# ShuoYangRobotics/Cerberus

Hardware: NVIDIA H100
Metric: sliding-window solves/sec (10-frame x 150-feature windows) (higher is better)
Workload: dtype f64

## Files before the change

cerberus_b200/csrc/solve_kernel.cuh:

```cuda
#pragma once
#include "eval_kernels.cuh"

namespace cerb {

#if defined(CERB_PHASE_TIMING) && !defined(CERB_CUSIM)
__device__ unsigned long long g_phase_cycles[48];
#define PH_DECL() long long ph_t = clock64()
#define PH_MARK_T(id, t) do { if ((threadIdx.x & 31) == 0) { const long long ph_n = clock64(); if (threadIdx.x == (t)) atomicAdd(&g_phase_cycles[id], (unsigned long long)(ph_n - ph_t)); ph_t = ph_n; } __syncwarp(); } while (0)
#define PH_MARK(id) PH_MARK_T(id, 0)
#define PH_ARG , long long &ph_t
#define PH_FWD , ph_t
#else
#define PH_DECL()
#define PH_MARK_T(id, t)
#define PH_MARK(id)
#define PH_ARG
#define PH_FWD
#endif

enum { CERB_WINDOW = 10, NX = 79, NYB = 13, NFR = 11, NY = 143, NR = 222, NRP = 224, HXX_SZ = 79 * 79, HXY_SZ = 79 * 143, X_TD = 78, SOLVE_THREADS = 256, FT = 64, TILE_LD = 33, NOBS_PLANES = 9 };
enum { HBLK = NYB * NYB, AD_SZ = NFR * HBLK, BO_SZ = (NFR - 1) * HBLK };
#ifndef CERB_SOLVE_MIN_BLOCKS
#define CERB_SOLVE_MIN_BLOCKS 1
#endif
enum { PIMG_HXY = HXX_SZ + 1, PIMG_REST = HXY_SZ + AD_SZ + BO_SZ, PIMG_SZ = PIMG_HXY + PIMG_REST, SMEM_HXX_PAD = 3 };
static_assert((PIMG_HXY * 8) % 16 == 0 && (PIMG_REST * 8) % 16 == 0 && ((HXX_SZ + SMEM_HXX_PAD) * 8) % 16 == 0, "bulk-copy alignment of the prior image");

struct SolveParams {
    int n_windows, maxF, maxObs, max_iters, optimize_leg_bias;
    double G[3], sqrt_info, huber;
    double radius0, max_radius, min_radius, min_rel_dec, ftol, gtol, ptol;
    const int *n_features, *feat_start, *feat_nobs, *feat_off, *flags;
    const double *obs; const int *obs_stereo;
    const double *pre;
    const double *sinfo;
    const double *prior_J, *prior_r, *prior_x0, *prior_Hp; const int *prior_meta;
    double *state, *lam;
    int *rep_i; double *rep_d;
    double *ws;
    long ws_stride;
    double *dbg; int dbg_window;
    double test_initial_mu;
    int no_bulk_copy;
    int test_fail_factorizations;
};

CERB_HD long ws_vecs(int F) { return (long)NX * F; }
CERB_HD long ws_prior(int F) { return (long)NX * F + 9L * F; }
CERB_HD long ws_chunks(int F) { return ws_prior(F) + PIMG_SZ; }
CERB_HD long ws_imuplan(int F) { return (ws_chunks(F) + (F + 4) / 2 + 8 + 1) & ~1L; }
CERB_HD long ws_size(int F) { return ws_imuplan(F) + 15 * 2 * 32 * 4 / 2 + 8; }
struct CtaWs {
    double *W, *hh, *gl, *sl, *Dl, *ghl, *gnl, *stl, *lamc, *sinv;
    int *chunks;
    int *imu_plan;
    double *pimg;
    int F;
};
CERB_D CtaWs ws_carve(const SolveParams &P) {
    double *ws = P.ws + (size_t)blockIdx.x * P.ws_stride;
    const int F = P.maxF;
    CtaWs v;
    v.W = ws;
    v.hh = ws + ws_vecs(F); v.gl = v.hh + F; v.sl = v.gl + F; v.Dl = v.sl + F; v.ghl = v.Dl + F; v.gnl = v.ghl + F; v.stl = v.gnl + F; v.lamc = v.stl + F; v.sinv = v.lamc + F;
    v.chunks = reinterpret_cast<int *>(ws + ws_chunks(F)); v.imu_plan = reinterpret_cast<int *>(ws + ws_imuplan(F));
    v.pimg = ws + ws_prior(F); v.F = F;
    return v;
}

struct Smem {
    double *Hxx, *Hxy, *Ad, *Bo;
    double *g, *sc, *D, *gh, *gn, *stp, *yv;
    double *xs, *xc;
    double *Rw, *Rex;
    double *Ju;
    double *lin;
    double *pdx, *pr;
    double *red;
    double *wj;
    double *sca;
    double *chain_col;
    double *idg;
    double *idx;
    int *ti;
    unsigned long long *mbar;
    double *tile;
};
enum { S_RADIUS = 0, S_MU, S_REUSE, S_XCOST, S_CCOST, S_ALPHA, S_GNORM2, S_GNNORM2, S_GDOTGN, S_MODEL, S_STEPNORM, S_XNORM, S_DLNORM,
       S_OK, S_DONE, S_TERM, S_ITER, S_NSUCC, S_INVALID, S_GMAX, S_INIT_COST, S_P, S_Q, S_VHV, S_LCOST, S_LNORM, S_LGMAX, S_COUNT };
static_assert(S_COUNT <= 32, "scalar slots overlap the chain's column line");
enum { TI_PRIOR_MAP = 0, TI_NCHUNKS = 96, TI_CHUNK_CACHE = 97, TI_CACHED_CHUNKS = 15, TI_CHAIN_DONE = 130, TI_IMU_MASK = 131, TI_INTS = 132 };
static_assert(TI_PRIOR_MAP + CERB_MAX_PRIOR_DIM <= TI_NCHUNKS && TI_CHUNK_CACHE + 2 * TI_CACHED_CHUNKS <= TI_CHAIN_DONE && TI_IMU_MASK < TI_INTS && TI_INTS % 2 == 0,
              "s.ti slots overlap");
enum { SMEM_DOUBLES = HXX_SZ + SMEM_HXX_PAD + HXY_SZ + AD_SZ + BO_SZ + 7 * NRP + 2 * ST_STRIDE + 99 + 18 + 3 + 31 * 39 + 960 + 192 + 8 * 256 + 128 * 8 + 32 + 32 + TI_INTS / 2 + 144 + 80 };

CERB_D void smem_carve(double *base, Smem &s) {
    double *p = base;
    s.Hxx = p; p += HXX_SZ; s.mbar = reinterpret_cast<unsigned long long *>(p + 1); p += SMEM_HXX_PAD; s.Hxy = p; p += HXY_SZ; s.Ad = p; p += AD_SZ; s.Bo = p; p += BO_SZ;
    s.g = p; p += NRP; s.sc = p; p += NRP; s.D = p; p += NRP; s.gh = p; p += NRP; s.gn = p; p += NRP; s.stp = p; p += NRP; s.yv = p; p += NRP;
    s.xs = p; p += ST_STRIDE; s.xc = p; p += ST_STRIDE;
    s.Rw = p; p += 99; s.Rex = p; p += 18; p += 3;
    s.Ju = p; p += 31 * 39; s.red = p; p += 8 * 256; s.wj = p; p += 128 * 8;
    s.lin = p; p += 960; s.pdx = p; p += 96; s.pr = p; p += 96; s.sca = p; p += 32; s.chain_col = p; p += 32;
    s.ti = reinterpret_cast<int *>(p); p += TI_INTS / 2;
    s.idg = p; p += 144;
    s.idx = p; p += 80;
    s.tile = s.Hxy;
}

template <int NV>
CERB_D void block_sum(const double *v, double *red, double *out, int tid) {
    for (int k = 0; k < NV; k++) red[k * 256 + tid] = v[k];
    __syncthreads();
    for (int s = 128; s > 0; s >>= 1) {
        if (tid < s) for (int k = 0; k < NV; k++) red[k * 256 + tid] += red[k * 256 + tid + s];
        __syncthreads();
    }
    for (int k = 0; k < NV; k++) out[k] = red[k * 256];
    __syncthreads();
}

CERB_D void copy_g2s(double *dst, const double *src, int n, int tid) {
    for (int k0 = tid; k0 < n; k0 += 8 * SOLVE_THREADS) {
        double b[8];
        _Pragma("unroll")
        for (int u = 0; u < 8; u++) { const int k = k0 + u * SOLVE_THREADS; b[u] = (k < n) ? src[k] : 0.0; }
        _Pragma("unroll")
        for (int u = 0; u < 8; u++) { const int k = k0 + u * SOLVE_THREADS; if (k < n) dst[k] = b[u]; }
    }
}
CERB_D void copy_g2s_async(double *dst, const double *src, int n, int tid) {
    for (int k = tid; k < n; k += SOLVE_THREADS) CERB_CP_ASYNC8(dst + k, src + k);
}
CERB_D void load_geometry(const double *x, Smem &s, int tid) {
    if (tid < 11) { const m33 R = qtoR(ldq(x + ST_POSE + 7 * tid + 3)); for (int k = 0; k < 9; k++) s.Rw[9 * tid + k] = R.m[k]; }
    else if (tid < 13) { const int e = tid - 11; const m33 R = qtoR(ldq(x + ST_EX + 7 * e + 3)); for (int k = 0; k < 9; k++) s.Rex[9 * e + k] = R.m[k]; }
    __syncthreads();
}

struct ObsCtx { int start, nobs, off; double lam, pix, piy, vix, viy, tdi; };

struct ObsVals { double px, py, vx, vy, td; int stereo; };
CERB_D void obs_fetch(const double *obs, const int *stereo, int mo, int o, int cam, ObsVals &v) {
    v.px = obs[(cam ? 4 : 0) * mo + o]; v.py = obs[(cam ? 5 : 1) * mo + o]; v.vx = obs[(cam ? 6 : 2) * mo + o]; v.vy = obs[(cam ? 7 : 3) * mo + o];
    v.td = obs[8 * mo + o]; v.stereo = stereo[o];
}

CERB_NOINLINE double vision_cost(const SolveParams &P, int w, const double *x, const double *lam, int tid) {
    CERB_DYN_SMEM(double, smem_base);
// ... 243 lines not shown
                        for (int ks = par; ks < nkt; ks += 2) {
                            const int rn = rb1 + 4 * (ks + 2 - par);
                            const bool more = ks + 2 < nkt;
                            const double n0 = more ? tq[0][rn] : 0.0, n1 = (more && !k3 && tv[1]) ? tq[1][rn] : 0.0, n2 = (more && tv[2]) ? tq[2][rn] : 0.0, n3 = (more && tv[3]) ? tq[3][rn] : 0.0;
                            CERB_DMMA(acc[0][0], acc[0][1], v0, v0, acc[0][0], acc[0][1]);
                            CERB_DMMA(acc[2][0], acc[2][1], v0, v2, acc[2][0], acc[2][1]);
                            CERB_DMMA(acc[3][0], acc[3][1], v0, v3, acc[3][0], acc[3][1]);
                            CERB_DMMA(acc[7][0], acc[7][1], v2, v2, acc[7][0], acc[7][1]);
                            CERB_DMMA(acc[8][0], acc[8][1], v2, v3, acc[8][0], acc[8][1]);
                            CERB_DMMA(acc[9][0], acc[9][1], v3, v3, acc[9][0], acc[9][1]);
                            if (!k3) {
                                CERB_DMMA(acc[1][0], acc[1][1], v0, v1, acc[1][0], acc[1][1]);
                                CERB_DMMA(acc[4][0], acc[4][1], v1, v1, acc[4][0], acc[4][1]);
                                CERB_DMMA(acc[5][0], acc[5][1], v1, v2, acc[5][0], acc[5][1]);
                                CERB_DMMA(acc[6][0], acc[6][1], v1, v3, acc[6][0], acc[6][1]);
                            }
                            v0 = n0; v1 = n1; v2 = n2; v3 = n3;
                        }
                    }
                    PH_MARK(28);
                    const int o = (lane >> 2) * 8 + 2 * (lane & 3);
                    pp[0 * 64 + o] += acc[0][0]; pp[0 * 64 + o + 1] += acc[0][1];
                    pp[1 * 64 + o] += acc[2][0]; pp[1 * 64 + o + 1] += acc[2][1];
                    pp[2 * 64 + o] += acc[3][0]; pp[2 * 64 + o + 1] += acc[3][1];
                    pp[3 * 64 + o] += acc[7][0]; pp[3 * 64 + o + 1] += acc[7][1];
                    pp[4 * 64 + o] += acc[8][0]; pp[4 * 64 + o + 1] += acc[8][1];
                    pp[5 * 64 + o] += acc[9][0]; pp[5 * 64 + o + 1] += acc[9][1];
                }
                {
                    const int o = wid * VJ_SZ + (lane >> 2) * 8 + 2 * (lane & 3);
                    jp[o] = acc[1][0]; jp[o + 1] = acc[1][1];
                    jp[64 + o] = acc[4][0]; jp[64 + o + 1] = acc[4][1];
                    jp[128 + o] = acc[5][0]; jp[128 + o + 1] = acc[5][1];
                    jp[192 + o] = acc[6][0]; jp[192 + o + 1] = acc[6][1];
                }
            }
            if (wrow && cam == 1) for (int k = 0; k < 6; k++) W[(size_t)(6 * j + k) * F + f] = wprev[k] + wjv[k] * (prescale ? s.sc[6 * j + k] * slf : 1.0);
            PH_MARK(29);
            __syncthreads();
            PH_MARK(22);
            if (jbase >= 0) {
                _Pragma("unroll")
                for (int fj = 0; fj < 2; fj++) {
                    const int jf = j0 + fj;
                    if (jf >= NFR || jf == a) continue;
                    const double *q = jp + (4 * fj) * VJ_SZ + tid;
                    smem_base[jbase + jca * a + jcj * jf] += ((q[0] + q[VJ_SZ]) + q[2 * VJ_SZ]) + q[3 * VJ_SZ];
                }
            }
            PH_MARK(23);
        }
        __syncthreads();
        {
            double *ex = T;
            ex[0 * 256 + tid] = h; ex[1 * 256 + tid] = gq; ex[2 * 256 + tid] = wT;
            for (int k = 0; k < 6; k++) { ex[(3 + k) * 256 + tid] = wI[k]; ex[(9 + k) * 256 + tid] = wE0[k]; ex[(15 + k) * 256 + tid] = wE1[k]; }
        }
        __syncthreads();
        for (int e = tid; e < VP_SZ; e += SOLVE_THREADS) {
            double v = 0.0;
            for (int wq = 0; wq < 8; wq++) v += ((wq < 5) ? s.Ju + 8 * VJ_SZ + VP_SZ * wq : s.tile + VT_SZ + VP_SZ * (wq - 5))[e];
            const int blk = e >> 6, ra = (e >> 3) & 7, rb = e & 7;
            const int ga = blk < 3 ? 0 : (blk < 5 ? 2 : 3), gb = blk == 0 ? 0 : (blk == 1 || blk == 3 ? 2 : 3);
            vis_scatter(s, ga, gb, ra, rb, a, a, v);
        }
        if (tid < 64 && ev) {
            const double *ex = T;
            double q[21];
            for (int k = 0; k < 21; k++) q[k] = ((ex[k * 256 + tid] + ex[k * 256 + 64 + tid]) + ex[k * 256 + 128 + tid]) + ex[k * 256 + 192 + tid];
            hh[f] = q[0] * slf * slf; gl[f] = q[1] * slf;
            W[(size_t)X_TD * F + f] = q[2] * (prescale ? s.sc[X_TD] * slf : 1.0);
            for (int k = 0; k < 6; k++) {
                W[(size_t)(6 * a + k) * F + f] = q[3 + k] * (prescale ? s.sc[6 * a + k] * slf : 1.0);
                W[(size_t)(66 + k) * F + f] = q[9 + k] * (prescale ? s.sc[66 + k] * slf : 1.0);
                W[(size_t)(72 + k) * F + f] = q[15 + k] * (prescale ? s.sc[72 + k] * slf : 1.0);
            }
        }
        __syncthreads();
        PH_MARK(24);
    }
    return cost;
}

CERB_D void imu_lin_all(const SolveParams &P, Smem &s, int w, const double *x, bool want_jac, int tid) {
    if (tid < CERB_WINDOW) {
        const double *pre = P.pre + ((size_t)w * CERB_WINDOW + tid) * PRE_STRIDE;
        IMULegLin *L = reinterpret_cast<IMULegLin *>(s.lin + 96 * tid);
        imu_leg_linearize(pre, x + ST_POSE + 7 * tid, x + ST_SB + 9 * tid, x + ST_LB + 4 * tid, x + ST_POSE + 7 * (tid + 1),
                          x + ST_SB + 9 * (tid + 1), x + ST_LB + 4 * (tid + 1), P.G, want_jac, L);
    }
    __syncthreads();
}

CERB_D double prior_residual(const SolveParams &P, Smem &s, int w, const double *x, int tid) {
    const int *meta = P.prior_meta + (size_t)w * PRIOR_META_STRIDE;
    if (!meta[0]) return 0.0;
    const int n = meta[1], nb = meta[2];
    const double *J = P.prior_J + (size_t)w * PRIOR_LD * PRIOR_LD, *r0 = P.prior_r + (size_t)w * PRIOR_LD, *x0 = P.prior_x0 + (size_t)w * 16 * 9;
    if (tid < nb) {
        const int kind = meta[4 + 3 * tid], index = meta[5 + 3 * tid], col = meta[6 + 3 * tid];
        prior_block_dx(kind, x + prior_block_state_offset(kind, index), x0 + 9 * tid, s.pdx + col);
    }
    __syncthreads();
    int parts = SOLVE_THREADS / n; if (parts > 4) parts = 4; if (parts < 1) parts = 1;
    const int kc = (n + parts - 1) / parts;
    double *part = s.red;
    for (int e = tid; e < parts * n; e += SOLVE_THREADS) {
        const int p = e / n, i = e % n;
        const int k1 = (p + 1) * kc < n ? (p + 1) * kc : n;
        double t = 0.0;
        for (int k = p * kc; k < k1; k++) t += J[(size_t)k * n + i] * s.pdx[k];
        part[p * PRIOR_LD + i] = t;
    }
    __syncthreads();
    double cost = 0.0;
    for (int i = tid; i < n; i += SOLVE_THREADS) {
        double t = r0[i];
        for (int p = 0; p < parts; p++) t += part[p * PRIOR_LD + i];
        s.pr[i] = t; cost += 0.5 * t * t;
    }
    __syncthreads();
    return cost;
}

CERB_NOINLINE double inertial_cost(const SolveParams &P, int w, const double *x, int tid) {
    CERB_DYN_SMEM(double, smem_base);
    Smem s; smem_carve(smem_base, s);
    imu_lin_all(P, s, w, x, false, tid);
    double cost = 0.0;
    for (int idx = tid; idx < CERB_WINDOW * 31; idx += SOLVE_THREADS) {
        const int i = idx / 31, r = idx % 31;
        const double *pre = P.pre + ((size_t)w * CERB_WINDOW + i) * PRE_STRIDE;
        if (pre[PRE_SUM_DT] > 10.0) continue;
        const double *ru = s.lin + 96 * i, *S = P.sinfo + ((size_t)w * CERB_WINDOW + i) * 961;
        double t = 0.0;
        for (int q = r; q < 31; q++) t += S[r * 31 + q] * ru[q];
        cost += 0.5 * t * t;
    }
    return cost + prior_residual(P, s, w, x, tid);
}

CERB_D int imu_col_dest(int i, int c) {
    if (c < 6) return 6 * i + c;
    if (c < 19) return -(1 + NYB * i + (c - 6));
    if (c < 25) return 6 * (i + 1) + (c - 19);
    return -(1 + NYB * (i + 1) + (c - 25));
}
CERB_D void scatter_addr(const Smem &s, int da, int db, double **a0, double **a1) {
    *a1 = nullptr;
    if (da >= 0 && db >= 0) { *a0 = (da <= db) ? s.Hxx + da * NX + db : s.Hxx + db * NX + da; return; }
    if (da >= 0) { *a0 = s.Hxy + da * NY + (-db - 1); return; }
    if (db >= 0) { *a0 = s.Hxy + db * NY + (-da - 1); return; }
    const int ya = -da - 1, yb = -db - 1;
    const int fa = ya / NYB, fb = yb / NYB, ka = ya % NYB, kb = yb % NYB;
    if (fa == fb) { *a0 = s.Ad + fa * HBLK + ka * NYB + kb; if (ka != kb) *a1 = s.Ad + fa * HBLK + kb * NYB + ka; }
    else if (fb == fa + 1) *a0 = s.Bo + fa * HBLK + ka * NYB + kb;
    else *a0 = s.Bo + fb * HBLK + kb * NYB + ka;
}
CERB_D void scatter_H(Smem &s, int da, int db, double v) {
    if (da >= 0 && db >= 0) { if (da <= db) s.Hxx[da * NX + db] += v; else s.Hxx[db * NX + da] += v; return; }
    if (da >= 0) { s.Hxy[da * NY + (-db - 1)] += v; return; }
    if (db >= 0) { s.Hxy[db * NY + (-da - 1)] += v; return; }
    const int ya = -da - 1, yb = -db - 1;
    const int fa = ya / NYB, fb = yb / NYB, ka = ya % NYB, kb = yb % NYB;
    if (fa == fb) { s.Ad[fa * HBLK + ka * NYB + kb] += v; if (ka != kb) s.Ad[fa * HBLK + kb * NYB + ka] += v; }
    else if (fb == fa + 1) s.Bo[fa * HBLK + ka * NYB + kb] += v;
    else s.Bo[fb * HBLK + kb * NYB + ka] += v;
}

enum { IMU_LDJ = 44, IMU_TILE = 32 * 44, IMU_WARPS = 3, PRIOR_THREADS = SOLVE_THREADS - 32 * IMU_WARPS };
CERB_NOINLINE double inertial_linearize(const SolveParams &P, int w, const double *x, int tid) {
    CERB_DYN_SMEM(double, smem_base);
    Smem s; smem_carve(smem_base, s);
    double cost = 0.0;
    PH_DECL();
    imu_lin_all(P, s, w, x, true, tid);
    PH_MARK(25);
    const int wid = tid >> 5, lane = tid & 31;
    CERB_CP_ASYNC_WAIT();
    double *gp = s.stp;
    double *ppart = s.yv;
    for (int k = tid; k < NRP; k += SOLVE_THREADS) gp[k] = 0.0;
    __syncthreads();
    if (wid < IMU_WARPS) {
        double *Jt = s.Ju + IMU_TILE * wid;
        int plx[30], ply[30];
        {
            const int *plan = ws_carve(P).imu_plan;
            _Pragma("unroll")
            for (int q = 0; q < 30; q++) { plx[q] = __ldg(plan + (2 * q) * 32 + lane); ply[q] = __ldg(plan + (2 * q + 1) * 32 + lane); }
            const int dummy = (int)(s.idg - smem_base) + lane;
            _Pragma("unroll")
            for (int q = 0; q < 30; q++) if (plx[q] == dummy && (ply[q] & 4095) == 0) plx[q] += 32 * wid;
        }
        double sa[20];
        auto load_S = [&](int i) {
            const double *S = P.sinfo + ((size_t)w * CERB_WINDOW + i) * 961;
            int q = 0;
            _Pragma("unroll")
            for (int mi = 0; mi < 4; mi++)
                _Pragma("unroll")
                for (int ks = 2 * mi; ks < 8; ks++) {
                    const int r = 8 * mi + (lane >> 2), c = 4 * ks + (lane & 3);
                    sa[q++] = (r < 31 && c < 31 && c >= r) ? S[r * 31 + c] : 0.0;
                }
        };
        load_S(wid * 4);
        const int imu_mask = s.ti[TI_IMU_MASK];
        double sdt[4];
        _Pragma("unroll")
        for (int rnd = 0; rnd < 4; rnd++) { const int i = rnd + 4 * wid; sdt[rnd] = (i < CERB_WINDOW) ? P.pre[((size_t)w * CERB_WINDOW + i) * PRE_STRIDE + PRE_SUM_DT] : 1e30; }
        _Pragma("unroll")
        for (int rnd = 0; rnd < 4; rnd++) {
            const int i = rnd + 4 * wid;
            const double *pre = P.pre + ((size_t)w * CERB_WINDOW + (i < CERB_WINDOW ? i : 0)) * PRE_STRIDE;
            if (i < CERB_WINDOW && !(sdt[rnd] > 10.0) && (imu_mask == 0 || (imu_mask == 1 && i == 0))) {
                for (int k = lane; k < IMU_TILE; k += 32) Jt[k] = 0.0;
                __syncwarp();
                if (lane < 11) imu_leg_fill_ju_part(*reinterpret_cast<const IMULegLin *>(s.lin + 96 * i), pre, Jt, IMU_LDJ, lane);
                if (lane < 31) Jt[lane * IMU_LDJ + 38] = s.lin[96 * i + lane];
                __syncwarp();
                PH_MARK(32);
                for (int ni = 0; ni < 5; ni++) {
                    double b[8];
                    _Pragma("unroll")
                    for (int ks = 0; ks < 8; ks++) b[ks] = Jt[(4 * ks + (lane & 3)) * IMU_LDJ + 8 * ni + (lane >> 2)];
                    __syncwarp();
                    double c[4][2];
                    int q = 0;
                    _Pragma("unroll")
                    for (int mi = 0; mi < 4; mi++) {
                        c[mi][0] = 0.0; c[mi][1] = 0.0;
                        _Pragma("unroll")
                        for (int ks = 2 * mi; ks < 8; ks++) { CERB_DMMA(c[mi][0], c[mi][1], sa[q], b[ks], c[mi][0], c[mi][1]); q++; }
                    }
                    _Pragma("unroll")
                    for (int mi = 0; mi < 4; mi++) { double *o = Jt + (8 * mi + (lane >> 2)) * IMU_LDJ + 8 * ni + 2 * (lane & 3); o[0] = c[mi][0]; o[1] = c[mi][1]; }
                    __syncwarp();
                }
                PH_MARK(33);
                if (i + 1 < CERB_WINDOW && rnd < 3) load_S(i + 1);
                double acc[15][2];
                _Pragma("unroll")
                for (int k = 0; k < 15; k++) { acc[k][0] = 0.0; acc[k][1] = 0.0; }
                for (int ks = 0; ks < 8; ks++) {
                    double f[5];
                    _Pragma("unroll")
                    for (int n = 0; n < 5; n++) f[n] = Jt[(4 * ks + (lane & 3)) * IMU_LDJ + 8 * n + (lane >> 2)];
                    int q = 0;
                    _Pragma("unroll")
                    for (int mi = 0; mi < 5; mi++)
                        _Pragma("unroll")
                        for (int ni = mi; ni < 5; ni++) { CERB_DMMA(acc[q][0], acc[q][1], f[mi], f[ni], acc[q][0], acc[q][1]); q++; }
                }
                PH_MARK(34);
                if (lane == 27) cost += 0.5 * acc[14][0];
                _Pragma("unroll")
                for (int hq = 0; hq < 30; hq += 15) {
                    double cur[15];
                    _Pragma("unroll")
                    for (int t = 0; t < 15; t++) cur[t] = smem_base[plx[hq + t] + i * (ply[hq + t] & 4095)];
                    _Pragma("unroll")
                    for (int t = 0; t < 15; t++) {
                        const int o = plx[hq + t] + i * (ply[hq + t] & 4095);
                        const double nv = cur[t] + acc[(hq + t) >> 1][(hq + t) & 1];
                        smem_base[o] = nv;
                        smem_base[o + (ply[hq + t] >> 12) - 256] = nv;
                    }
                }
                PH_MARK(35);
            } else if (i + 1 < CERB_WINDOW && rnd < 3) load_S(i + 1);
            CERB_BAR_SYNC(2, 32 * IMU_WARPS);
            PH_MARK(36);
        }
        PH_MARK(30);
    } else {
        const int *meta = P.prior_meta + (size_t)w * PRIOR_META_STRIDE;
        if (meta[0]) {
            const int t5 = tid - 32 * IMU_WARPS, n = meta[1], nb = meta[2];
            const double *J = P.prior_J + (size_t)w * PRIOR_LD * PRIOR_LD, *r0 = P.prior_r + (size_t)w * PRIOR_LD, *x0 = P.prior_x0 + (size_t)w * 16 * 9;
            if (t5 < nb) {
                const int kind = meta[4 + 3 * t5], index = meta[5 + 3 * t5], col = meta[6 + 3 * t5];
                prior_block_dx(kind, x + prior_block_state_offset(kind, index), x0 + 9 * t5, s.pdx + col);
            }
            CERB_BAR_SYNC(3, PRIOR_THREADS);
            const int kc = (n + 1) / 2;
            for (int e = t5; e < 2 * n; e += PRIOR_THREADS) {
                const int p = e / n, i = e % n;
                const int k1 = (p + 1) * kc < n ? (p + 1) * kc : n;
                double t = 0.0;
                for (int k = p * kc; k < k1; k++) t += J[(size_t)k * n + i] * s.pdx[k];
                ppart[p * PRIOR_LD + i] = t;
            }
            CERB_BAR_SYNC(3, PRIOR_THREADS);
            for (int i = t5; i < n; i += PRIOR_THREADS) {
                const double t = (r0[i] + ppart[i]) + ppart[PRIOR_LD + i];
                s.pr[i] = t; cost += 0.5 * t * t;
            }
            CERB_BAR_SYNC(3, PRIOR_THREADS);
            for (int c = wid - IMU_WARPS; c < n; c += PRIOR_THREADS / 32) {
                double t = 0.0;
                for (int k = lane; k < n; k += 32) t += J[(size_t)c * n + k] * s.pr[k];
                for (int o = 16; o > 0; o >>= 1) t += __shfl_sync(0xffffffffu, t, (lane + o) & 31);
                const int d = s.ti[TI_PRIOR_MAP + c];
                if (lane == 0) gp[d >= 0 ? d : NX + (-d - 1)] += t;
            }
        }
        PH_MARK_T(31, 96);
    }
    __syncthreads();
    PH_MARK(26);
    for (int k = tid; k < NR; k += SOLVE_THREADS) s.g[k] += gp[k];
    __syncthreads();
    PH_MARK(27);
    return cost;
}

CERB_D void apply_plus(const Smem &s, const double *delta, const double *lam, const double *dlam, double *lamc, int nF, bool ex_open, bool td_open, int tid) {
    if (tid < 11) pose_plus(s.xs + ST_POSE + 7 * tid, delta + 6 * tid, s.xc + ST_POSE + 7 * tid);
    else if (tid < 13) {
        const int e = tid - 11;
        if (ex_open) pose_plus(s.xs + ST_EX + 7 * e, delta + 66 + 6 * e, s.xc + ST_EX + 7 * e);
        else for (int k = 0; k < 7; k++) s.xc[ST_EX + 7 * e + k] = s.xs[ST_EX + 7 * e + k];
    }
    for (int k = tid; k < 99; k += SOLVE_THREADS) { const int f = k / 9, c = k % 9; s.xc[ST_SB + k] = s.xs[ST_SB + k] + delta[NX + NYB * f + c]; }
    for (int k = tid; k < 44; k += SOLVE_THREADS) { const int f = k / 4, c = k % 4; s.xc[ST_LB + k] = s.xs[ST_LB + k] + delta[NX + NYB * f + 9 + c]; }
    if (tid == 0) s.xc[ST_TD] = td_open ? s.xs[ST_TD] + delta[X_TD] : s.xs[ST_TD];
    for (int f = tid; f < nF; f += SOLVE_THREADS) lamc[f] = lam[f] + dlam[f];
    __syncthreads();
}

CERB_D double ambient_sq(const double *a, const double *b, const double *la, const double *lb, int nF, bool ex_open, bool lb_open, bool td_open, int tid) {
    double t = 0.0;
    for (int k = tid; k < ST_SIZE; k += SOLVE_THREADS) {
        if (k >= ST_LB && k < ST_EX && !lb_open) continue;
        if (k >= ST_EX && k < ST_TD && !ex_open) continue;
        if (k == ST_TD && !td_open) continue;
        const double v = b ? a[k] - b[k] : a[k];
        t += v * v;
    }
    for (int f = tid; f < nF; f += SOLVE_THREADS) { const double v = lb ? la[f] - lb[f] : la[f]; t += v * v; }
    return t;
}

template <bool SUB>
CERB_D double w_column_dot(const double *wf, int F, const double *v, double t) {
    constexpr int BATCH = 16;
    for (int a0 = 0; a0 < NX; a0 += BATCH) {
        double wr[BATCH];
        _Pragma("unroll")
        for (int u = 0; u < BATCH; u++) wr[u] = (a0 + u < NX) ? wf[(size_t)(a0 + u) * F] : 0.0;
        _Pragma("unroll")
        for (int u = 0; u < BATCH; u++) {
            if (a0 + u < NX) { if (SUB) t -= wr[u] * v[a0 + u]; else t += wr[u] * v[a0 + u]; }
        }
    }
    return t;
}

template <int W> struct TTPlan;
#define CERB_TT_PLAN(W, NR_, NB_, ...) template <> struct TTPlan<W> { static constexpr int nr = NR_, nb = NB_; static CERB_HD int tab(int i) { constexpr int t[] = {__VA_ARGS__}; return t[i]; } };
CERB_TT_PLAN(0, 4, 7, 0, 1, 2, 3, 0, 0, 0,   0, 0, 1, 0, 1, 0, 1,   0, 1, 1, 2, 2, 3, 3)
CERB_TT_PLAN(1, 4, 7, 2, 3, 4, 5, 0, 0, 0,   0, 0, 1, 0, 1, 0, 1,   0, 1, 1, 2, 2, 3, 3)
CERB_TT_PLAN(2, 4, 7, 4, 5, 6, 7, 0, 0, 0,   0, 0, 1, 0, 1, 0, 1,   0, 1, 1, 2, 2, 3, 3)
CERB_TT_PLAN(3, 4, 7, 6, 7, 8, 9, 0, 0, 0,   0, 0, 1, 0, 1, 0, 1,   0, 1, 1, 2, 2, 3, 3)
CERB_TT_PLAN(4, 6, 7, 8, 9, 0, 1, 4, 5, 0,   0, 0, 1, 2, 3, 2, 3,   0, 1, 1, 4, 4, 5, 5)
CERB_TT_PLAN(5, 6, 7, 0, 1, 6, 7, 8, 9, 0,   0, 0, 0, 0, 1, 1, 1,   2, 3, 4, 5, 2, 3, 4)
CERB_TT_PLAN(6, 7, 7, 1, 9, 2, 6, 7, 8, 3,   0, 2, 2, 2, 2, 6, 6,   1, 3, 4, 5, 1, 3, 4)
CERB_TT_PLAN(7, 5, 6, 3, 4, 5, 8, 9, 0, 0,   0, 0, 1, 1, 2, 2, 0,   3, 4, 3, 4, 3, 4, 0)
template <int W> CERB_D void ttt_warp(Smem &s, int lane) {
    typedef TTPlan<W> PL;
    const double *pr[7];
    _Pragma("unroll")
    for (int u = 0; u < 7; u++) {
        const int r = 8 * PL::tab(u < PL::nr ? u : 0) + (lane >> 2);
        pr[u] = (r < NX ? s.Hxy + r * NY : s.yv + NX) + (lane & 3);
    }
    double acc[7][2], fv[7];
    _Pragma("unroll")
    for (int k = 0; k < 7; k++) { acc[k][0] = 0.0; acc[k][1] = 0.0; }
    _Pragma("unroll")
    for (int u = 0; u < 7; u++) fv[u] = (u < PL::nr) ? pr[u][0] : 0.0;
    for (int q0 = 0; q0 < NY; q0 += 4) {
        const int qn = q0 + 4;
        const bool take = qn < NY && qn + (lane & 3) < NY;
        double fn[7];
        _Pragma("unroll")
        for (int u = 0; u < 7; u++) fn[u] = (u < PL::nr && take) ? pr[u][qn] : 0.0;
        _Pragma("unroll")
        for (int k = 0; k < 7; k++) if (k < PL::nb) CERB_DMMA(acc[k][0], acc[k][1], fv[PL::tab(7 + k)], fv[PL::tab(14 + k)], acc[k][0], acc[k][1]);
        _Pragma("unroll")
// ... 900 lines not shown
```

Before: 33730.

## Rebalance IMU factor work across four warps and batch prior gradient loads

Raises the IMU warp count from three to four, with a round-robin factor assignment so the ten IMU legs finish in three rounds instead of four. The tile stride shrinks to fit the extra tile. To make room, the per-leg linearization buffer moves from shared memory to the per-CTA global workspace. The prior-gradient J^T r loop now preloads four columns' worth of J values into registers before reducing, which increases memory-level parallelism but leaves fewer prior threads and adds global-memory traffic for the linearization data.

```diff
diff --git a/cerberus_b200/csrc/solve_kernel.cuh b/cerberus_b200/csrc/solve_kernel.cuh
--- a/cerberus_b200/csrc/solve_kernel.cuh
+++ b/cerberus_b200/csrc/solve_kernel.cuh
@@ -49,11 +49,13 @@
 CERB_HD long ws_prior(int F) { return (long)NX * F + 9L * F; }
 CERB_HD long ws_chunks(int F) { return ws_prior(F) + PIMG_SZ; }
 CERB_HD long ws_imuplan(int F) { return (ws_chunks(F) + (F + 4) / 2 + 8 + 1) & ~1L; }
-CERB_HD long ws_size(int F) { return ws_imuplan(F) + 15 * 2 * 32 * 4 / 2 + 8; }
+CERB_HD long ws_imulin(int F) { return ws_imuplan(F) + 15 * 2 * 32 * 4 / 2 + 8; }
+CERB_HD long ws_size(int F) { return ws_imulin(F) + 96 * 10; }
 struct CtaWs {
     double *W, *hh, *gl, *sl, *Dl, *ghl, *gnl, *stl, *lamc, *sinv;
     int *chunks;
     int *imu_plan;
+    double *imu_lin;
     double *pimg;
     int F;
 };
@@ -64,7 +66,7 @@
     v.W = ws;
     v.hh = ws + ws_vecs(F); v.gl = v.hh + F; v.sl = v.gl + F; v.Dl = v.sl + F; v.ghl = v.Dl + F; v.gnl = v.ghl + F; v.stl = v.gnl + F; v.lamc = v.stl + F; v.sinv = v.lamc + F;
     v.chunks = reinterpret_cast<int *>(ws + ws_chunks(F)); v.imu_plan = reinterpret_cast<int *>(ws + ws_imuplan(F));
-    v.pimg = ws + ws_prior(F); v.F = F;
+    v.pimg = ws + ws_prior(F); v.imu_lin = ws + ws_imulin(F); v.F = F;
     return v;
 }
 
@@ -474,10 +476,10 @@
     return cost;
 }
 
-CERB_D void imu_lin_all(const SolveParams &P, Smem &s, int w, const double *x, bool want_jac, int tid) {
+CERB_D void imu_lin_all(const SolveParams &P, double *lin, int w, const double *x, bool want_jac, int tid) {
     if (tid < CERB_WINDOW) {
         const double *pre = P.pre + ((size_t)w * CERB_WINDOW + tid) * PRE_STRIDE;
-        IMULegLin *L = reinterpret_cast<IMULegLin *>(s.lin + 96 * tid);
+        IMULegLin *L = reinterpret_cast<IMULegLin *>(lin + 96 * tid);
         imu_leg_linearize(pre, x + ST_POSE + 7 * tid, x + ST_SB + 9 * tid, x + ST_LB + 4 * tid, x + ST_POSE + 7 * (tid + 1),
                           x + ST_SB + 9 * (tid + 1), x + ST_LB + 4 * (tid + 1), P.G, want_jac, L);
     }
@@ -518,7 +520,7 @@
 CERB_NOINLINE double inertial_cost(const SolveParams &P, int w, const double *x, int tid) {
     CERB_DYN_SMEM(double, smem_base);
     Smem s; smem_carve(smem_base, s);
-    imu_lin_all(P, s, w, x, false, tid);
+    imu_lin_all(P, s.lin, w, x, false, tid);
     double cost = 0.0;
     for (int idx = tid; idx < CERB_WINDOW * 31; idx += SOLVE_THREADS) {
         const int i = idx / 31, r = idx % 31;
@@ -560,13 +562,21 @@
     else s.Bo[fb * HBLK + kb * NYB + ka] += v;
 }
 
-enum { IMU_LDJ = 44, IMU_TILE = 32 * 44, IMU_WARPS = 3, PRIOR_THREADS = SOLVE_THREADS - 32 * IMU_WARPS };
+enum { IMU_LDJ = 40, IMU_TILE = 32 * 40, IMU_WARPS = 4, IMU_ROUNDS = 3, PRIOR_THREADS = SOLVE_THREADS - 32 * IMU_WARPS };
+static_assert(IMU_WARPS * IMU_TILE <= 31 * 39 + 8 * 256 + 128 * 8 + 960, "the IMU tiles overrun Ju | red | wj | lin");
+static_assert(32 * IMU_WARPS <= 144, "the dummy slots of the IMU scatter overrun idg");
+CERB_D int imu_round_factor(int rnd, int wid) {
+    if (rnd == 0) return 2 * wid;
+    if (rnd == 1) return wid < 3 ? 2 * wid + 1 : 8;
+    return wid < 2 ? 7 + 2 * wid : -1;
+}
 CERB_NOINLINE double inertial_linearize(const SolveParams &P, int w, const double *x, int tid) {
     CERB_DYN_SMEM(double, smem_base);
     Smem s; smem_carve(smem_base, s);
     double cost = 0.0;
     PH_DECL();
-    imu_lin_all(P, s, w, x, true, tid);
+    double *lin = ws_carve(P).imu_lin;
+    imu_lin_all(P, lin, w, x, true, tid);
     PH_MARK(25);
     const int wid = tid >> 5, lane = tid & 31;
     CERB_CP_ASYNC_WAIT();
@@ -597,20 +607,21 @@
                     sa[q++] = (r < 31 && c < 31 && c >= r) ? S[r * 31 + c] : 0.0;
                 }
         };
-        load_S(wid * 4);
+        load_S(imu_round_factor(0, wid));
         const int imu_mask = s.ti[TI_IMU_MASK];
-        double sdt[4];
-        _Pragma("unroll")
-        for (int rnd = 0; rnd < 4; rnd++) { const int i = rnd + 4 * wid; sdt[rnd] = (i < CERB_WINDOW) ? P.pre[((size_t)w * CERB_WINDOW + i) * PRE_STRIDE + PRE_SUM_DT] : 1e30; }
-        _Pragma("unroll")
-        for (int rnd = 0; rnd < 4; rnd++) {
-            const int i = rnd + 4 * wid;
-            const double *pre = P.pre + ((size_t)w * CERB_WINDOW + (i < CERB_WINDOW ? i : 0)) * PRE_STRIDE;
-            if (i < CERB_WINDOW && !(sdt[rnd] > 10.0) && (imu_mask == 0 || (imu_mask == 1 && i == 0))) {
+        double sdt[IMU_ROUNDS];
+        _Pragma("unroll")
+        for (int rnd = 0; rnd < IMU_ROUNDS; rnd++) { const int i = imu_round_factor(rnd, wid); sdt[rnd] = (i >= 0) ? P.pre[((size_t)w * CERB_WINDOW + i) * PRE_STRIDE + PRE_SUM_DT] : 1e30; }
+        _Pragma("unroll")
+        for (int rnd = 0; rnd < IMU_ROUNDS; rnd++) {
+            const int i = imu_round_factor(rnd, wid);
+            const int inext = rnd + 1 < IMU_ROUNDS ? imu_round_factor(rnd + 1, wid) : -1;
+            const double *pre = P.pre + ((size_t)w * CERB_WINDOW + (i >= 0 ? i : 0)) * PRE_STRIDE;
+            if (i >= 0 && !(sdt[rnd] > 10.0) && (imu_mask == 0 || (imu_mask == 1 && i == 0))) {
                 for (int k = lane; k < IMU_TILE; k += 32) Jt[k] = 0.0;
                 __syncwarp();
-                if (lane < 11) imu_leg_fill_ju_part(*reinterpret_cast<const IMULegLin *>(s.lin + 96 * i), pre, Jt, IMU_LDJ, lane);
-                if (lane < 31) Jt[lane * IMU_LDJ + 38] = s.lin[96 * i + lane];
+                if (lane < 11) imu_leg_fill_ju_part(*reinterpret_cast<const IMULegLin *>(lin + 96 * i), pre, Jt, IMU_LDJ, lane);
+                if (lane < 31) Jt[lane * IMU_LDJ + 38] = lin[96 * i + lane];
                 __syncwarp();
                 PH_MARK(32);
                 for (int ni = 0; ni < 5; ni++) {
@@ -631,7 +642,7 @@
                     __syncwarp();
                 }
                 PH_MARK(33);
-                if (i + 1 < CERB_WINDOW && rnd < 3) load_S(i + 1);
+                if (inext >= 0) load_S(inext);
                 double acc[15][2];
                 _Pragma("unroll")
                 for (int k = 0; k < 15; k++) { acc[k][0] = 0.0; acc[k][1] = 0.0; }
@@ -661,7 +672,7 @@
                     }
                 }
                 PH_MARK(35);
-            } else if (i + 1 < CERB_WINDOW && rnd < 3) load_S(i + 1);
+            } else if (inext >= 0) load_S(inext);
             CERB_BAR_SYNC(2, 32 * IMU_WARPS);
             PH_MARK(36);
         }
@@ -690,15 +701,28 @@
                 s.pr[i] = t; cost += 0.5 * t * t;
             }
             CERB_BAR_SYNC(3, PRIOR_THREADS);
-            for (int c = wid - IMU_WARPS; c < n; c += PRIOR_THREADS / 32) {
-                double t = 0.0;
-                for (int k = lane; k < n; k += 32) t += J[(size_t)c * n + k] * s.pr[k];
-                for (int o = 16; o > 0; o >>= 1) t += __shfl_sync(0xffffffffu, t, (lane + o) & 31);
-                const int d = s.ti[TI_PRIOR_MAP + c];
-                if (lane == 0) gp[d >= 0 ? d : NX + (-d - 1)] += t;
-            }
-        }
-        PH_MARK_T(31, 96);
+            static_assert(PRIOR_LD <= 96, "three rows per lane");
+            enum { PW = PRIOR_THREADS / 32, PCOLS = 4 };
+            for (int c0 = wid - IMU_WARPS; c0 < n; c0 += PW * PCOLS) {
+                double v[PCOLS][3];
+                _Pragma("unroll")
+                for (int b = 0; b < PCOLS; b++)
+                    _Pragma("unroll")
+                    for (int q = 0; q < 3; q++) { const int c = c0 + PW * b, k = lane + 32 * q; v[b][q] = (c < n && k < n) ? J[(size_t)c * n + k] : 0.0; }
+                _Pragma("unroll")
+                for (int b = 0; b < PCOLS; b++) {
+                    const int c = c0 + PW * b;
+                    if (c >= n) break;
+                    double t = 0.0;
+                    _Pragma("unroll")
+                    for (int q = 0; q < 3; q++) if (lane + 32 * q < n) t += v[b][q] * s.pr[lane + 32 * q];
+                    for (int o = 16; o > 0; o >>= 1) t += __shfl_sync(0xffffffffu, t, (lane + o) & 31);
+                    const int d = s.ti[TI_PRIOR_MAP + c];
+                    if (lane == 0) gp[d >= 0 ? d : NX + (-d - 1)] += t;
+                }
+            }
+        }
+        PH_MARK_T(31, 32 * IMU_WARPS);
     }
     __syncthreads();
     PH_MARK(26);
```

New measurement: 34360, median of 6. +1.9%, better.

## Overlap prior residual with IMU linearization and split IMU factor work across warp pairs

Applied to the files above, without the earlier changes.

The IMU leg linearization (10 threads) now runs concurrently with the prior dx/J*dx computation on the other warps, in both the cost and linearize paths. That removes barriers and the serial dependency between the two. The IMU Gram/whitening work is split across pairs of warps (6 warps instead of 3), each half computing a subset of the DMMA tiles and synchronised with per-pair named barriers. The prior gradient J^T r is computed with 4 columns per warp iteration on the remaining 2 warps. The risks are more named-barrier traffic, higher register pressure from templated halves, and that only 2 warps are left for the prior gradient; the prior J^T r loop also assumes n <= 96.

```diff
diff --git a/cerberus_b200/csrc/solve_kernel.cuh b/cerberus_b200/csrc/solve_kernel.cuh
--- a/cerberus_b200/csrc/solve_kernel.cuh
+++ b/cerberus_b200/csrc/solve_kernel.cuh
@@ -474,51 +474,42 @@
     return cost;
 }
 
-CERB_D void imu_lin_all(const SolveParams &P, Smem &s, int w, const double *x, bool want_jac, int tid) {
-    if (tid < CERB_WINDOW) {
-        const double *pre = P.pre + ((size_t)w * CERB_WINDOW + tid) * PRE_STRIDE;
-        IMULegLin *L = reinterpret_cast<IMULegLin *>(s.lin + 96 * tid);
-        imu_leg_linearize(pre, x + ST_POSE + 7 * tid, x + ST_SB + 9 * tid, x + ST_LB + 4 * tid, x + ST_POSE + 7 * (tid + 1),
-                          x + ST_SB + 9 * (tid + 1), x + ST_LB + 4 * (tid + 1), P.G, want_jac, L);
-    }
-    __syncthreads();
-}
-
-CERB_D double prior_residual(const SolveParams &P, Smem &s, int w, const double *x, int tid) {
-    const int *meta = P.prior_meta + (size_t)w * PRIOR_META_STRIDE;
-    if (!meta[0]) return 0.0;
-    const int n = meta[1], nb = meta[2];
-    const double *J = P.prior_J + (size_t)w * PRIOR_LD * PRIOR_LD, *r0 = P.prior_r + (size_t)w * PRIOR_LD, *x0 = P.prior_x0 + (size_t)w * 16 * 9;
-    if (tid < nb) {
-        const int kind = meta[4 + 3 * tid], index = meta[5 + 3 * tid], col = meta[6 + 3 * tid];
-        prior_block_dx(kind, x + prior_block_state_offset(kind, index), x0 + 9 * tid, s.pdx + col);
-    }
-    __syncthreads();
-    int parts = SOLVE_THREADS / n; if (parts > 4) parts = 4; if (parts < 1) parts = 1;
-    const int kc = (n + parts - 1) / parts;
-    double *part = s.red;
-    for (int e = tid; e < parts * n; e += SOLVE_THREADS) {
-        const int p = e / n, i = e % n;
-        const int k1 = (p + 1) * kc < n ? (p + 1) * kc : n;
-        double t = 0.0;
-        for (int k = p * kc; k < k1; k++) t += J[(size_t)k * n + i] * s.pdx[k];
-        part[p * PRIOR_LD + i] = t;
-    }
-    __syncthreads();
-    double cost = 0.0;
-    for (int i = tid; i < n; i += SOLVE_THREADS) {
-        double t = r0[i];
-        for (int p = 0; p < parts; p++) t += part[p * PRIOR_LD + i];
-        s.pr[i] = t; cost += 0.5 * t * t;
-    }
-    __syncthreads();
-    return cost;
+CERB_D void imu_lin_thread(const SolveParams &P, Smem &s, int w, const double *x, bool want_jac, int tid) {
+    const double *pre = P.pre + ((size_t)w * CERB_WINDOW + tid) * PRE_STRIDE;
+    IMULegLin *L = reinterpret_cast<IMULegLin *>(s.lin + 96 * tid);
+    imu_leg_linearize(pre, x + ST_POSE + 7 * tid, x + ST_SB + 9 * tid, x + ST_LB + 4 * tid, x + ST_POSE + 7 * (tid + 1),
+                      x + ST_SB + 9 * (tid + 1), x + ST_LB + 4 * (tid + 1), P.G, want_jac, L);
+}
+CERB_D double prior_jdx_part(const double *J, int n, const double *dx, int i, int k0, int k1) {
+    double t = 0.0;
+    for (int k = k0; k < k1; k++) t += J[(size_t)k * n + i] * dx[k];
+    return t;
 }
 
 CERB_NOINLINE double inertial_cost(const SolveParams &P, int w, const double *x, int tid) {
     CERB_DYN_SMEM(double, smem_base);
     Smem s; smem_carve(smem_base, s);
-    imu_lin_all(P, s, w, x, false, tid);
+    const int *meta = P.prior_meta + (size_t)w * PRIOR_META_STRIDE;
+    const bool has_prior = meta[0] != 0;
+    const int n = meta[1];
+    int parts = has_prior ? SOLVE_THREADS / n : 1; if (parts > 4) parts = 4; if (parts < 1) parts = 1;
+    double *part = s.red;
+    if (tid < CERB_WINDOW) imu_lin_thread(P, s, w, x, false, tid);
+    else if (tid >= 32 && has_prior) {
+        const int t7 = tid - 32, nb = meta[2];
+        const double *J = P.prior_J + (size_t)w * PRIOR_LD * PRIOR_LD, *x0 = P.prior_x0 + (size_t)w * 16 * 9;
+        if (t7 < nb) {
+            const int kind = meta[4 + 3 * t7], index = meta[5 + 3 * t7], col = meta[6 + 3 * t7];
+            prior_block_dx(kind, x + prior_block_state_offset(kind, index), x0 + 9 * t7, s.pdx + col);
+        }
+        CERB_BAR_SYNC(3, SOLVE_THREADS - 32);
+        const int kc = (n + parts - 1) / parts;
+        for (int e = t7; e < parts * n; e += SOLVE_THREADS - 32) {
+            const int p = e / n, i = e % n;
+            part[p * PRIOR_LD + i] = prior_jdx_part(J, n, s.pdx, i, p * kc, (p + 1) * kc < n ? (p + 1) * kc : n);
+        }
+    }
+    __syncthreads();
     double cost = 0.0;
     for (int idx = tid; idx < CERB_WINDOW * 31; idx += SOLVE_THREADS) {
         const int i = idx / 31, r = idx % 31;
@@ -529,7 +520,17 @@
         for (int q = r; q < 31; q++) t += S[r * 31 + q] * ru[q];
         cost += 0.5 * t * t;
     }
-    return cost + prior_residual(P, s, w, x, tid);
+    double pcost = 0.0;
+    if (has_prior) {
+        const double *r0 = P.prior_r + (size_t)w * PRIOR_LD;
+        for (int i = tid; i < n; i += SOLVE_THREADS) {
+            double t = r0[i];
+            for (int p = 0; p < parts; p++) t += part[p * PRIOR_LD + i];
+            s.pr[i] = t; pcost += 0.5 * t * t;
+        }
+    }
+    __syncthreads();
+    return cost + pcost;
 }
 
 CERB_D int imu_col_dest(int i, int c) {
@@ -560,145 +561,171 @@
     else s.Bo[fb * HBLK + kb * NYB + ka] += v;
 }
 
-enum { IMU_LDJ = 44, IMU_TILE = 32 * 44, IMU_WARPS = 3, PRIOR_THREADS = SOLVE_THREADS - 32 * IMU_WARPS };
+enum { IMU_LDJ = 44, IMU_TILE = 32 * 44, IMU_PAIRS = 3, IMU_WARPS = 2 * IMU_PAIRS, PRIOR_COLS = 4 };
+static_assert(IMU_LDJ >= 42, "the per-warp dummy slots of the scatter plan are tile columns 40, 41");
+template <int H> struct ImuHalf { enum { NI0 = H ? 0 : 3, NI1 = H ? 3 : 5, Q0 = H ? 0 : 7, NQ = H ? 7 : 8 }; };
+CERB_HD constexpr int gram_mi(int q) { return q < 5 ? 0 : (q < 9 ? 1 : (q < 12 ? 2 : (q < 14 ? 3 : 4))); }
+CERB_HD constexpr int gram_ni(int q) { return q < 5 ? q : (q < 9 ? q - 4 : (q < 12 ? q - 7 : (q < 14 ? q - 9 : 4))); }
+
+template <int H>
+CERB_D double imu_factor_rounds(const SolveParams &P, Smem &s, double *smem_base, int w, int p, int lane) {
+    typedef ImuHalf<H> HF;
+    double cost = 0.0;
+    PH_DECL();
+    double *Jt = s.Ju + IMU_TILE * p;
+    const int pair_bar = 4 + p;
+    int plx[2 * HF::NQ], ply[2 * HF::NQ];
+    {
+        const int *plan = ws_carve(P).imu_plan;
+        _Pragma("unroll")
+        for (int q = 0; q < 2 * HF::NQ; q++) { plx[q] = __ldg(plan + (2 * (2 * HF::Q0 + q)) * 32 + lane); ply[q] = __ldg(plan + (2 * (2 * HF::Q0 + q) + 1) * 32 + lane); }
+        const int dummy = (int)(s.idg - smem_base) + lane, mine = (int)(Jt - smem_base) + lane * IMU_LDJ + 40 + H;
+        _Pragma("unroll")
+        for (int q = 0; q < 2 * HF::NQ; q++) if (plx[q] == dummy && (ply[q] & 4095) == 0) plx[q] = mine;
+    }
+    double sa[20];
+    auto load_S = [&](int i) {
+        const double *S = P.sinfo + ((size_t)w * CERB_WINDOW + i) * 961;
+        int q = 0;
+        _Pragma("unroll")
+        for (int mi = 0; mi < 4; mi++)
+            _Pragma("unroll")
+            for (int ks = 2 * mi; ks < 8; ks++) {
+                const int r = 8 * mi + (lane >> 2), c = 4 * ks + (lane & 3);
+                sa[q++] = (r < 31 && c < 31 && c >= r) ? S[r * 31 + c] : 0.0;
+            }
+    };
+    load_S(p * 4);
+    const int imu_mask = s.ti[TI_IMU_MASK];
+    double sdt[4];
+    _Pragma("unroll")
+    for (int rnd = 0; rnd < 4; rnd++) { const int i = rnd + 4 * p; sdt[rnd] = (i < CERB_WINDOW) ? P.pre[((size_t)w * CERB_WINDOW + i) * PRE_STRIDE + PRE_SUM_DT] : 1e30; }
+    _Pragma("unroll")
+    for (int rnd = 0; rnd < 4; rnd++) {
+        const int i = rnd + 4 * p;
+        const double *pre = P.pre + ((size_t)w * CERB_WINDOW + (i < CERB_WINDOW ? i : 0)) * PRE_STRIDE;
+        if (i < CERB_WINDOW && !(sdt[rnd] > 10.0) && (imu_mask == 0 || (imu_mask == 1 && i == 0))) {
+            for (int k = 32 * H + lane; k < IMU_TILE; k += 64) Jt[k] = 0.0;
+            CERB_BAR_SYNC(pair_bar, 64);
+            if (H == 0) { if (lane < 11) imu_leg_fill_ju_part(*reinterpret_cast<const IMULegLin *>(s.lin + 96 * i), pre, Jt, IMU_LDJ, lane); }
+            else if (lane < 31) Jt[lane * IMU_LDJ + 38] = s.lin[96 * i + lane];
+            CERB_BAR_SYNC(pair_bar, 64);
+            PH_MARK(32);
+            for (int ni = HF::NI0; ni < HF::NI1; ni++) {
+                double b[8];
+                _Pragma("unroll")
+                for (int ks = 0; ks < 8; ks++) b[ks] = Jt[(4 * ks + (lane & 3)) * IMU_LDJ + 8 * ni + (lane >> 2)];
+                __syncwarp();
+                double c[4][2];
+                int q = 0;
+                _Pragma("unroll")
+                for (int mi = 0; mi < 4; mi++) {
+                    c[mi][0] = 0.0; c[mi][1] = 0.0;
+                    _Pragma("unroll")
+                    for (int ks = 2 * mi; ks < 8; ks++) { CERB_DMMA(c[mi][0], c[mi][1], sa[q], b[ks], c[mi][0], c[mi][1]); q++; }
+                }
+                _Pragma("unroll")
+                for (int mi = 0; mi < 4; mi++) { double *o = Jt + (8 * mi + (lane >> 2)) * IMU_LDJ + 8 * ni + 2 * (lane & 3); o[0] = c[mi][0]; o[1] = c[mi][1]; }
+                __syncwarp();
+            }
+            PH_MARK(33);
+            if (i + 1 < CERB_WINDOW && rnd < 3) load_S(i + 1);
+            CERB_BAR_SYNC(pair_bar, 64);
+            double acc[HF::NQ][2];
+            _Pragma("unroll")
+            for (int k = 0; k < HF::NQ; k++) { acc[k][0] = 0.0; acc[k][1] = 0.0; }
+            for (int ks = 0; ks < 8; ks++) {
+                double f[5];
+                _Pragma("unroll")
+                for (int n = 0; n < 5; n++) f[n] = (H == 1 || n > 0) ? Jt[(4 * ks + (lane & 3)) * IMU_LDJ + 8 * n + (lane >> 2)] : 0.0;
+                _Pragma("unroll")
+                for (int k = 0; k < HF::NQ; k++) { CERB_DMMA(acc[k][0], acc[k][1], f[gram_mi(HF::Q0 + k)], f[gram_ni(HF::Q0 + k)], acc[k][0], acc[k][1]); }
+            }
+            PH_MARK(34);
+            if (H == 0 && lane == 27) cost += 0.5 * acc[14 - HF::Q0][0];
+            double cur[2 * HF::NQ];
+            _Pragma("unroll")
+            for (int t = 0; t < 2 * HF::NQ; t++) cur[t] = smem_base[plx[t] + i * (ply[t] & 4095)];
+            _Pragma("unroll")
+            for (int t = 0; t < 2 * HF::NQ; t++) {
+                const int o = plx[t] + i * (ply[t] & 4095);
+                const double nv = cur[t] + acc[t >> 1][t & 1];
+                smem_base[o] = nv;
+                smem_base[o + (ply[t] >> 12) - 256] = nv;
+            }
+            PH_MARK(35);
+        } else if (i + 1 < CERB_WINDOW && rnd < 3) load_S(i + 1);
+        CERB_BAR_SYNC(2, 32 * IMU_WARPS);
+        PH_MARK(36);
+    }
+    PH_MARK(30);
+    return cost;
+}
+
 CERB_NOINLINE double inertial_linearize(const SolveParams &P, int w, const double *x, int tid) {
     CERB_DYN_SMEM(double, smem_base);
     Smem s; smem_carve(smem_base, s);
     double cost = 0.0;
     PH_DECL();
-    imu_lin_all(P, s, w, x, true, tid);
+    const int wid = tid >> 5, lane = tid & 31;
+    const int *meta = P.prior_meta + (size_t)w * PRIOR_META_STRIDE;
+    const bool has_prior = meta[0] != 0;
+    const int n = meta[1];
+    const double *J = P.prior_J + (size_t)w * PRIOR_LD * PRIOR_LD;
+    double *gp = s.stp;
+    if (tid < CERB_WINDOW) imu_lin_thread(P, s, w, x, true, tid);
+    else if (wid > 0 && has_prior) {
+        const int t7 = tid - 32, nb = meta[2];
+        const double *r0 = P.prior_r + (size_t)w * PRIOR_LD, *x0 = P.prior_x0 + (size_t)w * 16 * 9;
+        double *ppart = s.yv;
+        if (t7 < nb) {
+            const int kind = meta[4 + 3 * t7], index = meta[5 + 3 * t7], col = meta[6 + 3 * t7];
+            prior_block_dx(kind, x + prior_block_state_offset(kind, index), x0 + 9 * t7, s.pdx + col);
+        }
+        CERB_BAR_SYNC(3, SOLVE_THREADS - 32);
+        const int kc = (n + 1) / 2;
+        for (int e = t7; e < 2 * n; e += SOLVE_THREADS - 32) {
+            const int p = e / n, i = e % n;
+            const int k1 = (p + 1) * kc < n ? (p + 1) * kc : n;
+            ppart[p * PRIOR_LD + i] = prior_jdx_part(J, n, s.pdx, i, p * kc, k1);
+        }
+        CERB_BAR_SYNC(3, SOLVE_THREADS - 32);
+        for (int i = tid - 96; i < n; i += SOLVE_THREADS - 96) {
+            if (i < 0) continue;
+            const double t = (r0[i] + ppart[i]) + ppart[PRIOR_LD + i];
+            s.pr[i] = t; cost += 0.5 * t * t;
+        }
+    }
+    CERB_CP_ASYNC_WAIT();
+    for (int k = tid; k < NRP; k += SOLVE_THREADS) gp[k] = 0.0;
+    __syncthreads();
     PH_MARK(25);
-    const int wid = tid >> 5, lane = tid & 31;
-    CERB_CP_ASYNC_WAIT();
-    double *gp = s.stp;
-    double *ppart = s.yv;
-    for (int k = tid; k < NRP; k += SOLVE_THREADS) gp[k] = 0.0;
-    __syncthreads();
     if (wid < IMU_WARPS) {
-        double *Jt = s.Ju + IMU_TILE * wid;
-        int plx[30], ply[30];
-        {
-            const int *plan = ws_carve(P).imu_plan;
-            _Pragma("unroll")
-            for (int q = 0; q < 30; q++) { plx[q] = __ldg(plan + (2 * q) * 32 + lane); ply[q] = __ldg(plan + (2 * q + 1) * 32 + lane); }
-            const int dummy = (int)(s.idg - smem_base) + lane;
-            _Pragma("unroll")
-            for (int q = 0; q < 30; q++) if (plx[q] == dummy && (ply[q] & 4095) == 0) plx[q] += 32 * wid;
-        }
-        double sa[20];
-        auto load_S = [&](int i) {
-            const double *S = P.sinfo + ((size_t)w * CERB_WINDOW + i) * 961;
-            int q = 0;
-            _Pragma("unroll")
-            for (int mi = 0; mi < 4; mi++)
+        cost += wid < IMU_PAIRS ? imu_factor_rounds<0>(P, s, smem_base, w, wid, lane) : imu_factor_rounds<1>(P, s, smem_base, w, wid - IMU_PAIRS, lane);
+    } else if (has_prior) {
+        for (int c0 = PRIOR_COLS * (wid - IMU_WARPS); c0 < n; c0 += PRIOR_COLS * (8 - IMU_WARPS)) {
+            double jv[PRIOR_COLS][3], t[PRIOR_COLS];
+            _Pragma("unroll")
+            for (int u = 0; u < PRIOR_COLS; u++)
                 _Pragma("unroll")
-                for (int ks = 2 * mi; ks < 8; ks++) {
-                    const int r = 8 * mi + (lane >> 2), c = 4 * ks + (lane & 3);
-                    sa[q++] = (r < 31 && c < 31 && c >= r) ? S[r * 31 + c] : 0.0;
-                }
-        };
-        load_S(wid * 4);
-        const int imu_mask = s.ti[TI_IMU_MASK];
-        double sdt[4];
-        _Pragma("unroll")
-        for (int rnd = 0; rnd < 4; rnd++) { const int i = rnd + 4 * wid; sdt[rnd] = (i < CERB_WINDOW) ? P.pre[((size_t)w * CERB_WINDOW + i) * PRE_STRIDE + PRE_SUM_DT] : 1e30; }
-        _Pragma("unroll")
-        for (int rnd = 0; rnd < 4; rnd++) {
-            const int i = rnd + 4 * wid;
-            const double *pre = P.pre + ((size_t)w * CERB_WINDOW + (i < CERB_WINDOW ? i : 0)) * PRE_STRIDE;
-            if (i < CERB_WINDOW && !(sdt[rnd] > 10.0) && (imu_mask == 0 || (imu_mask == 1 && i == 0))) {
-                for (int k = lane; k < IMU_TILE; k += 32) Jt[k] = 0.0;
-                __syncwarp();
-                if (lane < 11) imu_leg_fill_ju_part(*reinterpret_cast<const IMULegLin *>(s.lin + 96 * i), pre, Jt, IMU_LDJ, lane);
-                if (lane < 31) Jt[lane * IMU_LDJ + 38] = s.lin[96 * i + lane];
-                __syncwarp();
-                PH_MARK(32);
-                for (int ni = 0; ni < 5; ni++) {
-                    double b[8];
-                    _Pragma("unroll")
-                    for (int ks = 0; ks < 8; ks++) b[ks] = Jt[(4 * ks + (lane & 3)) * IMU_LDJ + 8 * ni + (lane >> 2)];
-                    __syncwarp();
-                    double c[4][2];
-                    int q = 0;
-                    _Pragma("unroll")
-                    for (int mi = 0; mi < 4; mi++) {
-                        c[mi][0] = 0.0; c[mi][1] = 0.0;
-                        _Pragma("unroll")
-                        for (int ks = 2 * mi; ks < 8; ks++) { CERB_DMMA(c[mi][0], c[mi][1], sa[q], b[ks], c[mi][0], c[mi][1]); q++; }
-                    }
-                    _Pragma("unroll")
-                    for (int mi = 0; mi < 4; mi++) { double *o = Jt + (8 * mi + (lane >> 2)) * IMU_LDJ + 8 * ni + 2 * (lane & 3); o[0] = c[mi][0]; o[1] = c[mi][1]; }
-                    __syncwarp();
-                }
-                PH_MARK(33);
-                if (i + 1 < CERB_WINDOW && rnd < 3) load_S(i + 1);
-                double acc[15][2];
+                for (int v = 0; v < 3; v++) { const int c = c0 + u, k = lane + 32 * v; jv[u][v] = (c < n && k < n) ? J[(size_t)c * n + k] : 0.0; }
+            _Pragma("unroll")
+            for (int u = 0; u < PRIOR_COLS; u++) {
+                t[u] = 0.0;
                 _Pragma("unroll")
-                for (int k = 0; k < 15; k++) { acc[k][0] = 0.0; acc[k][1] = 0.0; }
-                for (int ks = 0; ks < 8; ks++) {
-                    double f[5];
-                    _Pragma("unroll")
-                    for (int n = 0; n < 5; n++) f[n] = Jt[(4 * ks + (lane & 3)) * IMU_LDJ + 8 * n + (lane >> 2)];
-                    int q = 0;
-                    _Pragma("unroll")
-                    for (int mi = 0; mi < 5; mi++)
-                        _Pragma("unroll")
-                        for (int ni = mi; ni < 5; ni++) { CERB_DMMA(acc[q][0], acc[q][1], f[mi], f[ni], acc[q][0], acc[q][1]); q++; }
-                }
-                PH_MARK(34);
-                if (lane == 27) cost += 0.5 * acc[14][0];
+                for (int v = 0; v < 3; v++) if (lane + 32 * v < n) t[u] += jv[u][v] * s.pr[lane + 32 * v];
+            }
+            _Pragma("unroll")
+            for (int o = 16; o > 0; o >>= 1)
                 _Pragma("unroll")
-                for (int hq = 0; hq < 30; hq += 15) {
-                    double cur[15];
-                    _Pragma("unroll")
-                    for (int t = 0; t < 15; t++) cur[t] = smem_base[plx[hq + t] + i * (ply[hq + t] & 4095)];
-                    _Pragma("unroll")
-                    for (int t = 0; t < 15; t++) {
-                        const int o = plx[hq + t] + i * (ply[hq + t] & 4095);
-                        const double nv = cur[t] + acc[(hq + t) >> 1][(hq + t) & 1];
-                        smem_base[o] = nv;
-                        smem_base[o + (ply[hq + t] >> 12) - 256] = nv;
-                    }
-                }
-                PH_MARK(35);
-            } else if (i + 1 < CERB_WINDOW && rnd < 3) load_S(i + 1);
-            CERB_BAR_SYNC(2, 32 * IMU_WARPS);
-            PH_MARK(36);
-        }
-        PH_MARK(30);
-    } else {
-        const int *meta = P.prior_meta + (size_t)w * PRIOR_META_STRIDE;
-        if (meta[0]) {
-            const int t5 = tid - 32 * IMU_WARPS, n = meta[1], nb = meta[2];
-            const double *J = P.prior_J + (size_t)w * PRIOR_LD * PRIOR_LD, *r0 = P.prior_r + (size_t)w * PRIOR_LD, *x0 = P.prior_x0 + (size_t)w * 16 * 9;
-            if (t5 < nb) {
-                const int kind = meta[4 + 3 * t5], index = meta[5 + 3 * t5], col = meta[6 + 3 * t5];
-                prior_block_dx(kind, x + prior_block_state_offset(kind, index), x0 + 9 * t5, s.pdx + col);
-            }
-            CERB_BAR_SYNC(3, PRIOR_THREADS);
-            const int kc = (n + 1) / 2;
-            for (int e = t5; e < 2 * n; e += PRIOR_THREADS) {
-                const int p = e / n, i = e % n;
-                const int k1 = (p + 1) * kc < n ? (p + 1) * kc : n;
-                double t = 0.0;
-                for (int k = p * kc; k < k1; k++) t += J[(size_t)k * n + i] * s.pdx[k];
-                ppart[p * PRIOR_LD + i] = t;
-            }
-            CERB_BAR_SYNC(3, PRIOR_THREADS);
-            for (int i = t5; i < n; i += PRIOR_THREADS) {
-                const double t = (r0[i] + ppart[i]) + ppart[PRIOR_LD + i];
-                s.pr[i] = t; cost += 0.5 * t * t;
-            }
-            CERB_BAR_SYNC(3, PRIOR_THREADS);
-            for (int c = wid - IMU_WARPS; c < n; c += PRIOR_THREADS / 32) {
-                double t = 0.0;
-                for (int k = lane; k < n; k += 32) t += J[(size_t)c * n + k] * s.pr[k];
-                for (int o = 16; o > 0; o >>= 1) t += __shfl_sync(0xffffffffu, t, (lane + o) & 31);
-                const int d = s.ti[TI_PRIOR_MAP + c];
-                if (lane == 0) gp[d >= 0 ? d : NX + (-d - 1)] += t;
-            }
-        }
-        PH_MARK_T(31, 96);
+                for (int u = 0; u < PRIOR_COLS; u++) t[u] += __shfl_sync(0xffffffffu, t[u], (lane + o) & 31);
+            _Pragma("unroll")
+            for (int u = 0; u < PRIOR_COLS; u++) {
+                const int c = c0 + u;
+                if (c < n && lane == 0) { const int d = s.ti[TI_PRIOR_MAP + c]; gp[d >= 0 ? d : NX + (-d - 1)] += t[u]; }
+            }
+        }
+        PH_MARK_T(31, 32 * IMU_WARPS);
     }
     __syncthreads();
     PH_MARK(26);
```

After: 33670 before, 34670 after, median of 6. 1.03x the previous value.
